# CMU-Perceptual-Computing-Lab/caffe_rtpose

Measured on AMD Instinct MI355X. Metric: frames/sec (whole node) at 656x368 COCO model, higher is better.
Workload: dtype f16; 1 GPU; COCO 656x368, 1 scale(s), synthetic 720p video: pageable host u8 1280x720 frames through rtp_submit_frame: pinned copy + H2D + device warp / INTER_AREA / normalise / pad inside the timed region -> conv stack+ImResize+NMS+connect -> joints on the host; precision mode mixed, 7 frames in flight/GPU in ; precision=mixed, input=host_u8, batch_frames=2, frames_in_flight=7, num_scales=1, exec=graph, hw_queues=4, parallelism=frame-sharded replicas x1

## Files before the change

### caffe_rtpose_amd/csrc/conv_first.hip

```cpp
#include "conv_common.h"

namespace rtp {

namespace {
constexpr int FIRST_ZERO_SLOT = 8;
}

__global__ __launch_bounds__(256) void conv_first_kernel(FirstParams Q) {
  const KStamp kstamp_(Q.stamp);
  extern __shared__ __attribute__((aligned(16))) unsigned char smem_first[];
  _Float16* tile = (_Float16*)smem_first;
  const int W = Q.g.W, H = Q.g.H, TW = W + 2, TW3 = TW * 3;
  const int n = blockIdx.x / H, y = blockIdx.x - n * H;
  const int tid = threadIdx.x, lane = tid & 63, wave = tid >> 6;
  const int lpx = lane & 31, h = lane >> 5;
  const int zero_at = 3 * TW3;

  uint4 wa[2][2];
#pragma unroll
  for (int t = 0; t < 2; ++t)
#pragma unroll
    for (int j = 0; j < 2; ++j) wa[t][j] = Q.wfrag[(t * 2 + j) * 64 + lane];
  floatx16 bz[2];
#pragma unroll
  for (int t = 0; t < 2; ++t)
#pragma unroll
    for (int u = 0; u < 4; ++u) {
      const floatx4 b4 = *(const floatx4*)(Q.bias + t * 32 + (u >> 1) * 16 + h * 8 + (u & 1) * 4);
      bz[t][4 * u] = b4[0]; bz[t][4 * u + 1] = b4[1]; bz[t][4 * u + 2] = b4[2]; bz[t][4 * u + 3] = b4[3];
    }

  const float* img = Q.in + (long)n * 3 * H * W;
  for (int idx = tid; idx < 9 * W; idx += 256) {
    const int rc = idx / W, x = idx - rc * W;
    const int r = rc / 3, c = rc - r * 3;
    const int yy = y + r - 1;
    const float v = (yy >= 0 && yy < H) ? img[((long)c * H + yy) * W + x] : 0.f;
    tile[(r * TW + x + 1) * 3 + c] = (_Float16)v;
  }
  if (tid < 18) {
    const int r = tid / 6, rem = tid - r * 6, side = rem / 3, c = rem - side * 3;
    tile[(r * TW + (side ? W + 1 : 0)) * 3 + c] = (_Float16)0.f;
  }
  if (tid < FIRST_ZERO_SLOT) tile[zero_at + tid] = (_Float16)0.f;
  __syncthreads();

  int off[2][8], mul[2][8];
#pragma unroll
  for (int j = 0; j < 2; ++j)
#pragma unroll
    for (int e2 = 0; e2 < 8; ++e2) {
      const int k = j * 16 + h * 8 + e2;
      const bool real = k < 27;
      off[j][e2] = real ? (k / 9) * TW3 + (k % 9) : zero_at;
      mul[j][e2] = real ? 3 : 0;
    }

  _Float16* orow = Q.out + (((long)n * Q.g.Hp + y + Q.g.halo) * Q.g.Wp + Q.g.halo) * Q.Cp;
  for (int x0 = wave * 32; x0 < W; x0 += 128) {
    const int x = x0 + lpx;
    const int xr = x < W ? x : W - 1;
    half8_t b[2];
#pragma unroll
    for (int j = 0; j < 2; ++j)
#pragma unroll
      for (int e2 = 0; e2 < 8; ++e2) b[j][e2] = tile[xr * mul[j][e2] + off[j][e2]];
    floatx16 acc[2];
#pragma unroll
    for (int t = 0; t < 2; ++t) {
      acc[t] = __builtin_amdgcn_mfma_f32_32x32x16_f16(__builtin_bit_cast(half8_t, wa[t][0]), b[0], bz[t], 0, 0, 0);
      acc[t] = __builtin_amdgcn_mfma_f32_32x32x16_f16(__builtin_bit_cast(half8_t, wa[t][1]), b[1], acc[t], 0, 0, 0);
    }
    if (x < W) {
      _Float16* op = orow + (long)x * Q.Cp;
#pragma unroll
      for (int t = 0; t < 2; ++t)
#pragma unroll
        for (int g = 0; g < 2; ++g) {
          half8_t o;
#pragma unroll
          for (int u = 0; u < 8; ++u) {
            float v = acc[t][g * 8 + u];
            if (Q.relu) v = v > 0.f ? v : 0.f;
            o[u] = (_Float16)v;
          }
          *(half8_t*)(op + t * 32 + g * 16 + h * 8) = o;
        }
    }
  }
}

hipError_t launch_conv_first(const FirstParams& Q, hipStream_t stream) {
  const size_t lds = ((size_t)3 * (Q.g.W + 2) * 3 + FIRST_ZERO_SLOT) * sizeof(_Float16);
  if (lds > 64 * 1024) return hipErrorInvalidValue;
  hipLaunchKernelGGL(conv_first_kernel, dim3(Q.g.N * Q.g.H), dim3(256), lds, stream, Q);
  return hipGetLastError();
}

int conv_first_channel_of_row(int i) {
  const int hh = (i >> 2) & 1, q = (i & 3) + 4 * (i >> 3);
  return (q >> 3) * 16 + hh * 8 + (q & 7);
}

}
```

### caffe_rtpose_amd/csrc/engine.cpp

```cpp
#include <hip/hip_runtime.h>

#include <algorithm>
#include <atomic>
#include <chrono>
#include <cmath>
#include <cstdarg>
#include <cstdio>
#include <cstring>
#include <deque>
#include <fstream>
#include <map>
#include <mutex>
#include <sstream>
#include <string>
#include <thread>
#include <vector>

#include "../../include/rtpose_mi355x.h"
#include "jpeg_plan.h"
#include "kernels.h"
#include "netdef.h"
#include "plan.h"

using namespace rtp;
// ... 260 lines not shown
    for (int n = 0; n < c.cout; ++n) (*out_b)[n] = b[n];
    return;
  }
  if (c.fused) {
    const int rows = c.fused == 1 ? 128 : 64;
    const int parts = c.split_w ? 2 : 1;
    for (int n = 0; n < c.cout; ++n)
      for (int cr = 0; cr < c.cin; ++cr) {
        const int ci = ti.chmap[cr];
        const int chunk = c.fused == 1 ? n / 128 : ci / 128;
        const int row = c.fused == 1 ? n % 128 : n;
        const int k = ci % 128;
        const float wv = w[(size_t)n * c.cin + cr];
        const T hi = (T)wv;
        pw[(((size_t)chunk * parts + 0) * rows + row) * 128 + k] = hi;
        if (c.split_w) pw[(((size_t)chunk * parts + 1) * rows + row) * 128 + k] = (T)(wv - (float)hi);
      }
    out_b->assign(c.CoutP, 0.f);
    for (int n = 0; n < c.cout; ++n) (*out_b)[n] = b[n];
    return;
  }
  if (c.first) {
    for (int n = 0; n < c.cout; ++n)
      for (int r = 0; r < 3; ++r)
        for (int s = 0; s < 3; ++s)
          for (int cc = 0; cc < 3; ++cc) {
            const int j = (r * 3 + s) * 3 + cc;
            const int chunk = j / per_chunk, kk = j % per_chunk;
            const float wv = w[((size_t)(n * 3 + cc) * 3 + r) * 3 + s];
            const T hi = (T)wv;
            pw[((size_t)(0 * c.nchunk + chunk) * c.CoutP + n) * per_chunk + kpos(n, kk)] = hi;
            if (c.split_w) pw[((size_t)(0 * c.nchunk + c.ncp + chunk) * c.CoutP + n) * per_chunk + kpos(n, kk)] = (T)(wv - (float)hi);
          }
  } else {
    for (int n = 0; n < c.cout; ++n)
      for (int cr = 0; cr < c.cin; ++cr) {
        const int ci = ti.chmap[cr];
        const int chunk = ci / per_chunk, kk = ci % per_chunk;
        for (int r = 0; r < c.k; ++r)
          for (int s = 0; s < c.k; ++s) {
            const int tap = r * c.k + s;
            const float wv = w[((size_t)(n * c.cin + cr) * c.k + r) * c.k + s];
            const T hi = (T)wv;
            const T lo = (T)(wv - (float)hi);
            if (c.h8) {
              const size_t tile0 = (size_t)(r * c.nchunk + chunk) * c.k + s;
              pw[(tile0 * c.CoutP + n) * per_chunk + kpos(n, kk)] = hi;
              const size_t tileq = (size_t)(r * c.nchunk + c.ncp + chunk) * c.k + s;
              unsigned char* qrow = out_w->data() + (tileq * c.CoutP + n) * c.rowb;
              const int g = kk / 64, pos = kk % 64;
              auto qpos = [&](int byte) { return ((byte / 16) ^ conv_ring_swz(c.rowb, n)) * 16 + byte % 16; };
              qrow[qpos(g * 128 + pos)] = f32_to_e4m3(std::ldexp((float)hi, c.wq_exp));
              qrow[qpos(g * 128 + 64 + pos)] = f32_to_e4m3(std::ldexp(wv - (float)hi, c.wq_exp + 11));
              continue;
            }
            int vbase = 0;
            for (int pass = 0; pass < 3; ++pass) {
              if ((pass == 1 && !c.split_a) || (pass == 2 && !c.split_w)) continue;
              const int vchunk = vbase + chunk;
              vbase += c.ncp;
              const size_t tile = c.impl == 1 ? ((size_t)(r * c.nchunk + vchunk) * c.k + s) : ((size_t)tap * c.nchunk + vchunk);
              pw[(tile * c.CoutP + n) * per_chunk + kpos(n, kk)] = pass == 2 ? lo : hi;
            }
          }
      }
  }
  out_b->assign(c.CoutP, 0.f);
  for (int n = 0; n < c.cout; ++n) (*out_b)[n] = b[n];
}

void compute_wq_exp(rtp_engine* e) {
  for (auto& s : e->plan.steps) {
    if (s.type != 1 || !e->plan.convs[s.a].h8) continue;
    float mx = 0.f;
    for (int idx : {s.a, s.b}) if (idx >= 0) for (float v : e->w_ref[idx]) mx = std::max(mx, std::fabs(v));
    int ex = mx > 0.f ? (int)std::floor(std::log2(448.0 / mx)) : 0;
    ex = std::max(-20, std::min(ex, 40));
    for (int idx : {s.a, s.b}) if (idx >= 0) e->plan.convs[idx].wq_exp = ex;
  }
}

int upload_conv_weights(rtp_engine* e, int i) {
  const ConvOp& c = e->plan.convs[i];
  std::vector<unsigned char> pw;
  std::vector<float> pb;
  if (e->plan.prec == 0) pack_conv<_Float16>(e->plan, c, e->w_ref[i], e->b_ref[i], &pw, &pb);
  else pack_conv<float>(e->plan, c, e->w_ref[i], e->b_ref[i], &pw, &pb);
  SYNC_GUARD;
  HIPCHK(e, hipMemcpy(e->dweights + c.w_off, pw.data(), pw.size(), hipMemcpyHostToDevice));
  HIPCHK(e, hipMemcpy(e->dweights + c.b_off, pb.data(), pb.size() * sizeof(float), hipMemcpyHostToDevice));
  return RTP_OK;
}

int upload_all_weights(rtp_engine* e) {
  std::vector<unsigned char> image(e->plan.weights_bytes, 0);
  const int n = (int)e->plan.convs.size();
  const int nthr = std::max(1, std::min({(int)std::thread::hardware_concurrency(), 16, n}));
  std::atomic<int> next{0};
  auto work = [&]() {
    std::vector<unsigned char> pw;
    std::vector<float> pb;
    for (int i = next.fetch_add(1); i < n; i = next.fetch_add(1)) {
      const ConvOp& c = e->plan.convs[i];
      if (e->plan.prec == 0) pack_conv<_Float16>(e->plan, c, e->w_ref[i], e->b_ref[i], &pw, &pb);
      else pack_conv<float>(e->plan, c, e->w_ref[i], e->b_ref[i], &pw, &pb);
      memcpy(image.data() + c.w_off, pw.data(), pw.size());
      memcpy(image.data() + c.b_off, pb.data(), pb.size() * sizeof(float));
    }
  };
  std::vector<std::thread> pool;
  for (int t = 1; t < nthr; ++t) pool.emplace_back(work);
  work();
  for (auto& t : pool) t.join();
  SYNC_GUARD;
  HIPCHK(e, hipMemcpy(e->dweights, image.data(), e->plan.weights_bytes, hipMemcpyHostToDevice));
  return RTP_OK;
}

constexpr int STAMP_SLOTS = 256;
unsigned long long* stamp_slot(const rtp_engine* e, const Ctx& cx, int idx) {
  return (e->stamp_probe && cx.stamps && idx >= 0 && idx < STAMP_SLOTS) ? cx.stamps + 2 * (size_t)idx : nullptr;
}
int stamp_harvest(rtp_engine* e, Ctx& cx) {
  if (!cx.stamps || !cx.stamps_dirty) return RTP_OK;
  for (Slot& sl : cx.slot)
    if (sl.export_pending) HIPCHK(e, hipEventSynchronize(sl.ev_export));
  std::vector<unsigned long long> h(2 * STAMP_SLOTS);
  HIPCHK(e, hipMemcpy(h.data(), cx.stamps, h.size() * sizeof(unsigned long long), hipMemcpyDeviceToHost));
  HIPCHK(e, hipMemset(cx.stamps, 0, h.size() * sizeof(unsigned long long)));
  cx.stamps_dirty = false;
  for (int i = 0; i < STAMP_SLOTS; ++i) {
    if (!h[2 * i + 1] || !h[2 * i]) continue;
    const unsigned long long t0 = ~h[2 * i], t1 = h[2 * i + 1];
    if (!e->stamp_base) e->stamp_base = t0;
    if (e->stamp_spans.size() < 3 * (size_t)(1 << 20)) {
      e->stamp_spans.push_back((float)i);
      e->stamp_spans.push_back((float)((double)((long long)(t0 - e->stamp_base)) * 0.01));
      e->stamp_spans.push_back((float)((double)((long long)(t1 - e->stamp_base)) * 0.01));
    }
  }
  return RTP_OK;
}

void fill_problem(const rtp_engine* e, const Ctx& cx, const ConvOp& c, ConvProblem* pr) {
  memset(pr, 0, sizeof(*pr));
  pr->in = cx.arena + e->plan.tensors[c.in_tensor].offset;
  pr->w = e->dweights + c.w_off;
  pr->bias = (const float*)(e->dweights + c.b_off);
  pr->ndst = (int)c.dsts.size();
  for (int d = 0; d < pr->ndst; ++d) {
    const Tensor& t = e->plan.tensors[c.dsts[d].first];
    pr->dst[d].base = cx.arena + t.offset;
    pr->dst[d].cstride = t.stride();
    pr->dst[d].coff = c.dsts[d].second;
    pr->dst[d].lo_off = t.lo_off();
    pr->dst[d].q_off = t.q_off();
  }
  if (c.to_lowres) {
    pr->out_nchw = cx.lowres;
    pr->out_C = e->plan.heat_channels;
    pr->out_coff = c.lowres_coff;
  }
  pr->Cout = c.cout;
}

unsigned long long* g_clkprobe = nullptr;
int launch_conv_step(rtp_engine* e, Ctx& cx, const Step& s, int nimg) {
  const ConvOp& A = e->plan.convs[s.a];
  const Geom& g = e->plan.geom[A.level];
  ConvParams P;
  memset(&P, 0, sizeof P);
  fill_problem(e, cx, A, &P.prob[0]);
  if (s.b >= 0) fill_problem(e, cx, e->plan.convs[s.b], &P.prob[1]);
  P.H = g.H; P.W = g.W; P.Wp = g.Wp; P.halo = g.halo; P.img_pix = g.img_pix;
  P.in_cstride = e->plan.tensors[A.in_tensor].stride();
  P.nchunk = A.nchunk;
  P.wrap_at = A.wrap_at();
  P.last_phys = A.last_phys();
  {
    const Tensor& tin = e->plan.tensors[A.in_tensor];
    const int qb = tin.q_off() * e->plan.elem;
    P.q_from = A.h8 ? A.ncp : 0;
    P.jump_delta = A.h8 ? qb - (A.ncp - 1) * A.rowb : 0;
    P.row_back = A.h8 ? qb + (A.ncp - 1) * A.rowb : A.last_phys() * A.rowb;
    P.wq_exp = A.wq_exp;
  }
  P.CoutP = A.CoutP;
  P.tiles_per_img = (int)conv_tiles_per_img(e->plan, A);
  if (A.pool >= 0) {
    const Geom& go = e->plan.geom[A.level + 1];
    P.pool = 1;
    P.pool_wq = pool_wq(g, A);
    P.pool_Wp = go.Wp; P.pool_halo = go.halo; P.pool_img_pix = go.img_pix;
  }
  P.relu = A.relu ? 1 : 0;
  P.clkprobe = g_clkprobe;
  P.stamp = stamp_slot(e, cx, (int)(&s - e->plan.steps.data()));
  P.nimg = nimg;
  {
    static const char* rot = RTP_EXP_ENV("RTP_CONV_ROTATE");
    P.rotate = (rot && rot[0] == '0') ? 0 : 1;
    static const char* xm = RTP_EXP_ENV("RTP_CONV_XCDMAP");
    P.xcdmap = xm ? atoi(xm) : 1;
    static const char* sb = RTP_EXP_ENV("RTP_RING_SB");
    P.ring_sb = sb ? atoi(sb) : 6;
    static const char* sp = RTP_EXP_ENV("RTP_RING_SPEC");
    P.spec = (sp && sp[0] == '0') ? 0 : 1;
    static const char* rv = RTP_EXP_ENV("RTP_RING_VAR");
    P.variant = rv ? atoi(rv) : 0;
    static const char* ed = RTP_EXP_ENV("RTP_EPI_DIAG");
    P.diag = ed ? atoi(ed) : 0;
    static const char* il = RTP_EXP_ENV("RTP_RING_ILV");
    P.ilv = il ? (il[0] == '1' || (il[0] == 'q' && A.h8) || (il[0] == '7' && A.h8 && A.k_eff == 7)) : (A.h8 ? 1 : 0);
  }
  if (A.impl == 1) HIPCHK(e, launch_conv_ring(e->plan.prec, A.cfg, A.k_eff, A.rowb, P, s.b >= 0 ? 2 : 1, nimg, cx.stream));
  else HIPCHK(e, launch_conv(e->plan.prec, A.cfg, A.k_eff, A.rowb, P, s.b >= 0 ? 2 : 1, nimg, cx.stream));
  return RTP_OK;
}

int launch_pw2_step(rtp_engine* e, Ctx& cx, const Step& s, int nimg) {
  const ConvOp& A = e->plan.convs[s.a];
  const ConvOp& C = e->plan.convs[s.a2];
  const Geom& g = e->plan.geom[C.level];
  Pw2Params Q;
  memset(&Q, 0, sizeof Q);
  ConvParams& P = Q.P2;
  fill_problem(e, cx, C, &P.prob[0]);
  if (s.b2 >= 0) fill_problem(e, cx, e->plan.convs[s.b2], &P.prob[1]);
  P.H = g.H; P.W = g.W; P.Wp = g.Wp; P.halo = g.halo; P.img_pix = g.img_pix;
  P.CoutP = 64;
  P.tiles_per_img = (int)plain_tiles_per_img(g, 64);
  P.relu = C.relu ? 1 : 0;
  P.stamp = stamp_slot(e, cx, (int)(&s - e->plan.steps.data()));
  P.nimg = nimg;
  const int firsts[2] = {s.a, s.b};
  for (int q = 0; q < 2; ++q) {
    if (firsts[q] < 0) continue;
    const ConvOp& F = e->plan.convs[firsts[q]];
    const Tensor& ti = e->plan.tensors[F.in_tensor];
    const Tensor& tm = e->plan.tensors[F.dsts[0].first];
    Q.x_in[q] = cx.arena + ti.offset;
    Q.x_cstride = ti.stride();
    Q.x_lo_off = F.split_a ? ti.lo_off() : 0;
    Q.w1[q] = e->dweights + F.w_off;
    Q.b1[q] = (const float*)(e->dweights + F.b_off);
    Q.mid[q].base = tm.written ? cx.arena + tm.offset : nullptr;
    Q.mid[q].cstride = tm.stride();
    Q.mid[q].coff = 0;
    Q.mid[q].lo_off = tm.lo_off();
  }
  Q.c1_chunks = A.fused_chunks;
  Q.relu1 = A.relu ? 1 : 0;
  Q.split_w1 = A.split_w ? 1 : 0;
  Q.split_w2 = C.split_w ? 1 : 0;
  Q.h_lo = C.split_a ? 1 : 0;
  static const char* probe = RTP_EXP_ENV("RTP_PW2_PROBE");
  static int probed = 0;
  hipStreamCaptureStatus cst = hipStreamCaptureStatusNone;
  if (probe) (void)hipStreamIsCapturing(cx.stream, &cst);
  if (probe && cst == hipStreamCaptureStatusNone && probed < 16) {
    unsigned long long* d = nullptr;
    HIPCHK(e, hipMalloc((void**)&d, 32 * 8));
    HIPCHK(e, hipMemset(d, 0, 32 * 8));
    P.clkprobe = d;
    const auto t0 = std::chrono::steady_clock::now();
    HIPCHK(e, launch_conv_pw2(Q, s.b >= 0 ? 2 : 1, nimg, cx.stream));
    HIPCHK(e, hipStreamSynchronize(cx.stream));
    const double host_us = std::chrono::duration<double, std::micro>(std::chrono::steady_clock::now() - t0).count();
    unsigned long long h[32];
    HIPCHK(e, hipMemcpy(h, d, sizeof h, hipMemcpyDeviceToHost));
    (void)hipFree(d);
    fprintf(stderr, "pw2 probe %s chunks %d splits %d%d%d%d (launch+sync %.1f us): ", A.name.c_str(), Q.c1_chunks, Q.x_lo_off ? 1 : 0, Q.split_w1, Q.h_lo, Q.split_w2, host_us);
    for (unsigned i = 2; i <= h[0] && i < 32; ++i) fprintf(stderr, "%.2f ", (double)(h[i] - h[i - 1]) / 100.0);
    fprintf(stderr, "us; total %.2f us\n", (double)(h[h[0]] - h[1]) / 100.0);
    ++probed;
    return RTP_OK;
  }
  HIPCHK(e, launch_conv_pw2(Q, s.b >= 0 ? 2 : 1, nimg, cx.stream));
  return RTP_OK;
}

}

namespace {
bool is_dominant_class(const rtp_engine* e, const Step& s) {
  if (s.type != 1 || e->plan.dominant_step < 0) return false;
  const ConvOp& a = e->plan.convs[s.a];
  const ConvOp& d = e->plan.convs[e->plan.steps[e->plan.dominant_step].a];
  return a.k == d.k && a.cin == d.cin && a.cout == d.cout && (s.b >= 0) == (e->plan.steps[e->plan.dominant_step].b >= 0);
}

int launch_first_step(rtp_engine* e, Ctx& cx, const Step& s, const float* input_dev, int nimg) {
  const ConvOp& c = e->plan.convs[s.a];
  const Tensor& to = e->plan.tensors[c.dsts[0].first];
  FirstParams Q;
  Q.in = input_dev;
  Q.g = e->plan.geom[0];
  Q.g.N = nimg;
  Q.wfrag = (const uint4*)(e->dweights + c.w_off);
  Q.bias = (const float*)(e->dweights + c.b_off);
  Q.out = (_Float16*)(cx.arena + to.offset);
  Q.Cp = to.stride();
  Q.relu = c.relu ? 1 : 0;
  Q.stamp = stamp_slot(e, cx, (int)(&s - e->plan.steps.data()));
  HIPCHK(e, launch_conv_first(Q, cx.stream));
  return RTP_OK;
}

int run_frame_stack(rtp_engine* e, Ctx& cx, const float* input_dev, int nimg, bool cap = false) {
  const std::vector<PoolOp>& pools = e->plan.pools;
  auto geom_n = [&](int level) { Geom g = e->plan.geom[level]; g.N = nimg; return g; };
  for (size_t si = 0; si < e->plan.steps.size(); ++si) {
    const Step& s = e->plan.steps[si];
    const bool want_timed = e->time_dominant && !cap && nimg == e->plan.NI && (e->time_all || is_dominant_class(e, s));
    const bool timed = want_timed && e->tev_next < (int)e->tev.size() / 2;
    if (want_timed && !timed) e->probe_dropped[0]++;
    if (timed) HIPCHK(e, hipEventRecord(e->tev[2 * (size_t)e->tev_next], cx.stream));
    struct Close {
      rtp_engine* e; Ctx& cx; const Step& s; size_t si; bool timed;
      ~Close() {
        if (!timed) return;
        (void)hipEventRecord(e->tev[2 * (size_t)e->tev_next + 1], cx.stream);
        e->tev_step[e->tev_next] = (short)si;
        e->tev_pass[e->tev_next++] = (unsigned char)(s.type == 1 ? e->plan.convs[s.a].passes() : 1);
      }
    } close_{e, cx, s, si, timed};
    if (s.type == 0) {
      const Tensor& t = e->plan.tensors[0];
      HIPCHK(e, launch_pack_input(e->plan.prec, input_dev, cx.arena + t.offset, geom_n(0), t.stride(), cx.stream));
    } else if (s.type == 1) {
      const int rc = launch_conv_step(e, cx, s, nimg);
      if (rc) return rc;
    } else if (s.type == 3) {
      const int rc = launch_pw2_step(e, cx, s, nimg);
      if (rc) return rc;
    } else if (s.type == 4) {
      const int rc = launch_first_step(e, cx, s, input_dev, nimg);
      if (rc) return rc;
    } else {
      const PoolOp& p = pools[s.a];
      const Tensor& ti = e->plan.tensors[p.in_tensor];
      const Tensor& to = e->plan.tensors[p.out_tensor];
      HIPCHK(e, launch_maxpool(e->plan.prec, cx.arena + ti.offset, geom_n(ti.level), ti.stride(), cx.arena + to.offset, geom_n(to.level), to.stride(),
                               round_up(p.C, 16 / e->plan.elem), ti.lo_off(), to.lo_off(), ti.q_off(), to.q_off(), cx.stream));
    }
  }
  return RTP_OK;
}

ResizeParams resize_params(rtp_engine* e, Ctx& cx, int sj) {
  Slot& sl = cx.slot[sj];
  ResizeParams rp;
  rp.src = cx.lowres + (size_t)sj * e->N * e->plan.heat_channels * e->plan.low_h * e->plan.low_w;
  rp.dst = sl.resized; rp.num = e->N; rp.C = e->plan.heat_channels;
  rp.h = e->plan.low_h; rp.w = e->plan.low_w; rp.tw = e->cfg.net_w; rp.th = e->cfg.net_h;
  rp.start_scale = e->start_scale; rp.scale_gap = e->scale_gap;
  return rp;
}
int run_resize(rtp_engine* e, Ctx& cx, int sj = 0) {
  HIPCHK(e, launch_resize(resize_params(e, cx, sj), cx.slot[sj].stream));
  return RTP_OK;
}
NmsParams nms_params(rtp_engine* e, Ctx& cx, int sj) {
  Slot& sl = cx.slot[sj];
  NmsParams np;
  np.src = sl.resized; np.peaks = sl.peaks; np.strip_count = sl.strip_count; np.strip_list = sl.strip_list;
  np.src_planes = e->plan.heat_channels; np.H = e->cfg.net_h; np.W = e->cfg.net_w; np.num_parts = e->plan.num_parts;
  np.max_peaks = e->plan.max_peaks; np.nstrips = e->plan.nstrips; np.strip_rows = e->plan.strip_rows; np.threshold = e->nms_threshold;
  np.probe = nullptr;
  np.clear_flag = nullptr;
  np.stamp = stamp_slot(e, cx, 64 + 8 * sj);
  return np;
}
int run_nms(rtp_engine* e, Ctx& cx, int sj = 0) {
  HIPCHK(e, launch_nms(nms_params(e, cx, sj), cx.slot[sj].stream));
  return RTP_OK;
}
ConnectParams connect_params(rtp_engine* e, Ctx& cx, int sj) {
  Slot& sl = cx.slot[sj];
  ConnectParams cp;
  memset(&cp, 0, sizeof cp);
  cp.heat = sl.resized; cp.peaks = sl.peaks; cp.joints = sl.joints; cp.num_people = sl.num_people;
  cp.cand_score = sl.cand_score; cp.cand_ij = sl.cand_ij; cp.cand_count = sl.cand_count; cp.cand_blk = sl.cand_blk;
  cp.conn = sl.conn; cp.conn_score = sl.conn_score; cp.conn_count = sl.conn_count;
  cp.max_rows = e->plan.max_rows; cp.model = e->plan.model; cp.num_parts = e->plan.num_parts; cp.num_limbs = e->plan.num_limbs;
  cp.max_peaks = e->plan.max_peaks; cp.net_w = e->cfg.net_w; cp.net_h = e->cfg.net_h; cp.disp_w = e->cfg.disp_w; cp.disp_h = e->cfg.disp_h;
  cp.inter_threshold = e->inter_threshold; cp.inter_min_above = e->inter_min_above; cp.min_subset_cnt = e->min_subset_cnt;
  cp.min_subset_score = e->min_subset_score; cp.max_people = RTP_MAX_PEOPLE;
  cp.stamp = stamp_slot(e, cx, 64 + 8 * sj + 2);
  {
    static const char* pf = RTP_EXP_ENV("RTP_PAIRS_FULL");
    cp.pairs_full = (pf && pf[0] == '1') ? 1 : 0;
  }
  return cp;
}
int run_connect(rtp_engine* e, Ctx& cx, int sj = 0) {
  HIPCHK(e, launch_connect(connect_params(e, cx, sj), cx.slot[sj].stream));
  return RTP_OK;
}
int run_post_fused(rtp_engine* e, Ctx& cx, int sj, hipEvent_t ev_nms) {
  Slot& sl = cx.slot[sj];
  const ResizeParams rp = resize_params(e, cx, sj);
  NmsParams np = nms_params(e, cx, sj);
  np.clear_flag = sl.num_people;
  HIPCHK(e, launch_nms_fused(np, rp, sl.stream));
  HIPCHK(e, hipEventRecord(ev_nms, sl.stream));
  ConnectParams cp = connect_params(e, cx, sj);
  cp.counter_cleared = 1;
  cp.tickets = e->chain_connect ? sl.tickets : nullptr;
  HIPCHK(e, launch_connect_fused(cp, rp, sl.stream));
  return RTP_OK;
}

int jpeg_alloc(rtp_engine* e, int w, int h, JpegBufs* b, unsigned char** host, unsigned char** host_dev, size_t* cap);
void jd_free(JdBufs* b);
int jd_launch(rtp_engine* e, unsigned long long* stamp, const JdJob& job, const FrameView& dst, hipStream_t stream);

int launch_batch_body(rtp_engine* e, Ctx& cx, int nframes, const float* input_dev, bool materialize, bool cap, int part = 3) {
  int rc;
  if (part & 1) {
    HIPCHK(e, hipEventRecord(cx.ev[0], cx.stream));
    if ((rc = run_frame_stack(e, cx, input_dev, nframes * e->N, cap))) return rc;
  }
  if (!(part & 2)) return RTP_OK;
  HIPCHK(e, hipEventRecord(cx.ev[1], cx.stream));
  const size_t jbytes = (size_t)RTP_MAX_PEOPLE * e->plan.num_parts * 3 * sizeof(float);
  for (int j = 0; j < nframes; ++j) {
    Slot& sl = cx.slot[j];
    if (sl.stream != cx.stream) HIPCHK(e, hipStreamWaitEvent(sl.stream, cx.ev[1], 0));
    static const char* diag = RTP_EXP_ENV("RTP_DIAG_SKIP_POST");
    const int skip = diag ? atoi(diag) : 0;
    static const char* unf = RTP_EXP_ENV("RTP_POST_UNFUSED");
    HIPCHK(e, hipEventRecord(sl.ev[0], sl.stream));
    if (skip >= 3) {
      const ResizeParams rp = resize_params(e, cx, j);
      HIPCHK(e, hipEventRecord(sl.ev[1], sl.stream));
      HIPCHK(e, launch_nms_fused(nms_params(e, cx, j), rp, sl.stream));
      HIPCHK(e, hipEventRecord(sl.ev[2], sl.stream));
      if (skip >= 4) {
        ConnectParams cp = connect_params(e, cx, j);
        cp.diag_stages = skip - 3;
        HIPCHK(e, launch_connect_fused(cp, rp, sl.stream));
      }
    } else if (materialize || skip || (unf && unf[0] == '1')) {
      if (skip < 2 && (rc = run_resize(e, cx, j))) return rc;
      HIPCHK(e, hipEventRecord(sl.ev[1], sl.stream));
      if (skip < 2 && (rc = run_nms(e, cx, j))) return rc;
      HIPCHK(e, hipEventRecord(sl.ev[2], sl.stream));
      if (skip < 1 && (rc = run_connect(e, cx, j))) return rc;
    } else {
      HIPCHK(e, hipEventRecord(sl.ev[1], sl.stream));
      if ((rc = run_post_fused(e, cx, j, sl.ev[2]))) return rc;
    }
    HIPCHK(e, hipEventRecord(sl.ev[3], sl.stream));
    if (e->cfg.render && sl.has_disp) {
      const size_t dbytes = (size_t)e->cfg.disp_w * e->cfg.disp_h * 3;
      if (!sl.render_dev) {
        SYNC_GUARD;
        HIPCHK(e, hipMalloc((void**)&sl.render_dev, dbytes));
        HIPCHK(e, hipHostMalloc((void**)&sl.render_host, dbytes, hipHostMallocDefault));
        HIPCHK(e, hipMalloc((void**)&sl.render_tab, render_tab_floats(RTP_MAX_PEOPLE) * sizeof(float)));
      }
      if (e->cfg.render == 1) {
        RenderParams rp;
        rp.src = sl.disp_cur; rp.dst = sl.render_dev; rp.w = e->cfg.disp_w; rp.h = e->cfg.disp_h;
        rp.poses = sl.joints; rp.num_people = sl.num_people; rp.tab = sl.render_tab;
        rp.model = e->plan.model; rp.googly = 0; rp.max_people = RTP_MAX_PEOPLE;
        HIPCHK(e, launch_render(rp, sl.stream));
      } else {
        if (!(materialize || skip || (unf && unf[0] == '1')) && (rc = run_resize(e, cx, j))) return rc;
        RenderViewParams vp;
        vp.src = sl.disp_cur; vp.dst = sl.render_dev; vp.w = e->cfg.disp_w; vp.h = e->cfg.disp_h;
        vp.maps = sl.resized; vp.net_w = e->cfg.net_w; vp.net_h = e->cfg.net_h;
        vp.model = e->plan.model; vp.part_to_show = e->cfg.render - 1;
        HIPCHK(e, launch_render_view(vp, sl.stream));
      }
      if (e->jpeg_quality) {
        if (!sl.jpeg.base) {
          SYNC_GUARD;
          if ((rc = jpeg_alloc(e, e->cfg.disp_w, e->cfg.disp_h, &sl.jpeg, &sl.jpeg_host, &sl.jpeg_host_dev, &sl.jpeg_cap))) return rc;
        }
        const FrameView fv = {sl.render_dev, e->cfg.disp_w, e->cfg.disp_h, 3L * e->cfg.disp_w, 3L, {0L, 1L, 2L}};
        HIPCHK(e, launch_jpeg_encode(stamp_slot(e, cx, 64 + 8 * j + 6), fv, e->jpeg_q, sl.jpeg, sl.jpeg_host_dev,
                                     reinterpret_cast<unsigned*>(sl.jpeg_host_dev + sl.jpeg_cap), sl.stream));
      } else {
        if (!sl.render_host) {
          SYNC_GUARD;
          HIPCHK(e, hipHostMalloc((void**)&sl.render_host, dbytes, hipHostMallocDefault));
        }
        HIPCHK(e, hipMemcpyAsync(sl.render_host, sl.render_dev, dbytes, hipMemcpyDeviceToHost, sl.stream));
      }
    }
    HIPCHK(e, hipMemcpyAsync(sl.host_out + 4, sl.joints, jbytes, hipMemcpyDeviceToHost, sl.stream));
    HIPCHK(e, hipMemcpyAsync(sl.host_out, sl.num_people, sizeof(int), hipMemcpyDeviceToHost, sl.stream));
    HIPCHK(e, hipEventRecord(sl.ev[4], sl.stream));
    if (cap && sl.stream != cx.stream) HIPCHK(e, hipStreamWaitEvent(cx.stream, sl.ev[4], 0));
  }
  return RTP_OK;
}

int capture_batch(rtp_engine* e, Ctx& cx, int nframes, hipGraphExec_t* out) {
  SYNC_GUARD;
  hipGraph_t g = nullptr;
  HIPCHK(e, hipStreamBeginCapture(cx.stream, hipStreamCaptureModeThreadLocal));
  const int rc = launch_batch_body(e, cx, nframes, cx.input, false, true, e->graph_post ? 3 : 1);
  const hipError_t s = hipStreamEndCapture(cx.stream, &g);
  if (rc) { if (g) (void)hipGraphDestroy(g); return rc; }
  if (s != hipSuccess || !g) return fail(e, RTP_EHIP, "hipStreamEndCapture failed: %s", hipGetErrorString(s));
  const hipError_t si = hipGraphInstantiate(out, g, nullptr, nullptr, 0);
  (void)hipGraphDestroy(g);
  if (si != hipSuccess) return fail(e, RTP_EHIP, "hipGraphInstantiate failed: %s", hipGetErrorString(si));
  return RTP_OK;
}

int flush_prep(rtp_engine* e, Ctx& cx, bool force);
int launch_batch(rtp_engine* e, Ctx& cx, int nframes, const float* input_dev, bool materialize = false) {
  int rc;
  cx.last_nframes = nframes;
  cx.last_own_input = input_dev == cx.input;
  cx.last_tags.resize(nframes);
  for (int j = 0; j < nframes; ++j) cx.last_tags[j] = cx.slot[j].tag;
  for (Slot& sl : cx.slot)
    if (sl.export_pending) {
      HIPCHK(e, hipStreamWaitEvent(cx.stream, sl.ev_export, 0));
      sl.export_pending = false;
    }
  if (e->prep_defer && (rc = flush_prep(e, cx, true))) return rc;
  if (cx.in_pending) {
    if (cx.in_stream != cx.stream) {
      HIPCHK(e, hipEventRecord(cx.ev_in, cx.in_stream));
      HIPCHK(e, hipStreamWaitEvent(cx.stream, cx.ev_in, 0));
    }
    cx.in_pending = false;
  }
  static const char* diag = RTP_EXP_ENV("RTP_DIAG_SKIP_POST");
  static const char* unf = RTP_EXP_ENV("RTP_POST_UNFUSED");
  const bool graph = e->use_graph && !e->time_dominant && !materialize && input_dev == cx.input && !e->cfg.render && !diag && !unf && nframes <= 16;
  cx.graph_run = graph;
  cx.graph_conv = false;
  if (!graph) {
    if ((rc = launch_batch_body(e, cx, nframes, input_dev, materialize, false))) return rc;
    cx.launched = true;
    return RTP_OK;
  }
  if (!cx.gexec[nframes] && (rc = capture_batch(e, cx, nframes, &cx.gexec[nframes]))) return rc;
  HIPCHK(e, hipEventRecord(cx.gev[0], cx.stream));
  HIPCHK(e, hipGraphLaunch(cx.gexec[nframes], cx.stream));
  if (!e->graph_post) {
    if ((rc = launch_batch_body(e, cx, nframes, cx.input, false, false, 2))) return rc;
    cx.graph_run = false;
    cx.graph_conv = true;
  }
  HIPCHK(e, hipEventRecord(cx.gev[1], cx.stream));
  cx.launched = true;
  return RTP_OK;
}
int enqueue_frame(rtp_engine* e, Ctx& cx, const float* input_dev, bool materialize = false) { return launch_batch(e, cx, 1, input_dev, materialize); }

int hw_queue_count() {
  const char* v = getenv("GPU_MAX_HW_QUEUES");
  const int q = v ? atoi(v) : 4;
  return q >= 1 && q <= 64 ? q : 4;
}
hipError_t make_stream(hipStream_t* s, bool post) {
#ifdef RTP_EXPERIMENTS
  if (post) {
    const char* c = getenv("RTP_POST_CUS");
    const int n = c ? atoi(c) : 0;
    if (n > 0 && n < 256) {
      uint32_t mask[8] = {0, 0, 0, 0, 0, 0, 0, 0};
      for (int b = 0; b < n; ++b) mask[b >> 5] |= 1u << (b & 31);
      return hipExtStreamCreateWithCUMask(s, 8, mask);
    }
  }
  const char* v = getenv(post ? "RTP_POST_PRIO" : "RTP_CONV_PRIO");
  if (v && v[0]) {
    int least = 0, greatest = 0;
    (void)hipDeviceGetStreamPriorityRange(&least, &greatest);
    int pr = atoi(v);
    pr = std::max(greatest, std::min(least, pr));
    return hipStreamCreateWithPriority(s, hipStreamNonBlocking, pr);
  }
#endif
  (void)post;
  return hipStreamCreateWithFlags(s, hipStreamNonBlocking);
}

size_t staged_yuv_bytes(int w, int h, int sx, int sy, size_t* planes_off) {
  const size_t off = round_up_sz((size_t)w * h * 3, 256);
  if (planes_off) *planes_off = off;
  return off + (size_t)w * h + 2 * (size_t)((w + sx) >> sx) * (size_t)((h + sy) >> sy);
}

int alloc_slot(rtp_engine* e, Ctx& cx, Slot& sl, bool share_stream) {
  if (sl.preset_stream) {}
  else if (share_stream) sl.stream = cx.stream;
  else { HIPCHK(e, make_stream(&sl.stream, true)); sl.own_stream = true; }
  const size_t res_floats = (size_t)e->plan.heat_channels * e->cfg.net_h * e->cfg.net_w;
  HIPCHK(e, hipMalloc((void**)&sl.resized, res_floats * sizeof(float)));
  const size_t peak_floats = (size_t)e->plan.num_parts * (e->plan.max_peaks + 1) * 3;
  HIPCHK(e, hipMalloc((void**)&sl.peaks, peak_floats * sizeof(float)));
  HIPCHK(e, hipMemset(sl.peaks, 0, peak_floats * sizeof(float)));
  HIPCHK(e, hipMalloc((void**)&sl.strip_count, (size_t)e->plan.num_parts * e->plan.nstrips * sizeof(int)));
  HIPCHK(e, hipMalloc((void**)&sl.strip_list, (size_t)e->plan.num_parts * e->plan.nstrips * e->plan.max_peaks * sizeof(int)));
  const size_t pairs = (size_t)e->plan.num_limbs * e->plan.max_peaks * e->plan.max_peaks;
  HIPCHK(e, hipMalloc((void**)&sl.cand_score, pairs * sizeof(float)));
// ... 2573 lines not shown
```

### caffe_rtpose_amd/csrc/kernels.h

```cpp
#pragma once
#include <hip/hip_runtime.h>
#include <stdint.h>
#include <stdlib.h>

#include "jpeg_bound.h"
#include "jpeg_dec.h"

#ifdef RTP_EXPERIMENTS
#define RTP_EXP_ENV(name) getenv(name)
#else
#define RTP_EXP_ENV(name) ((const char*)nullptr)
#endif

namespace rtp {

#if defined(__HIPCC__)
struct KStamp {
  unsigned long long* s;
  __device__ __forceinline__ explicit KStamp(unsigned long long* p) : s(p) {
    if (s && threadIdx.x == 0 && threadIdx.y == 0) atomicMax(s, ~wall_clock64());
  }
  __device__ __forceinline__ ~KStamp() {
    if (s && threadIdx.x == 0 && threadIdx.y == 0) atomicMax(s + 1, wall_clock64());
  }
};
#endif

struct Geom {
  int N, H, W, halo, Hp, Wp;
  long img_pix;
};

#define RTP_MAX_DST 6
struct ConvDst {
  void* base;
  int cstride;
  int coff;
  int lo_off;
  int q_off;
};

struct ConvProblem {
  const void* in;
  const void* w;
  const float* bias;
  ConvDst dst[RTP_MAX_DST];
  int ndst;
  float* out_nchw;
  int out_C, out_coff;
  int Cout;
};

struct ConvParams {
  ConvProblem prob[2];
  int H, W, Wp, halo;
  long img_pix;
  int in_cstride;
  int nchunk;
  int wrap_at;
  int last_phys;
  int q_from;
  int wq_exp;
  int jump_delta;
  int row_back;
  int CoutP;
  int tiles_per_img;
  int nimg;
  int relu;
  int rotate;
  int xcdmap;
  int ring_sb;
  int spec;
  int variant;
  int ilv;
  int pool, pool_wq, pool_Wp, pool_halo;
  long pool_img_pix;
  int diag;
  unsigned long long* stamp;
  unsigned long long* clkprobe;
};

enum ConvCfg { CFG_128x128 = 0, CFG_64x128 = 1, CFG_64x64 = 2, CFG_128x64 = 3, CFG_128x32 = 4, CFG_256x64 = 5, CFG_COUNT = 6 };

struct ConvCfgInfo { int BM, BN; };
inline ConvCfgInfo conv_cfg_info(int cfg) {
  switch (cfg) {
    case CFG_128x128: return {128, 128};
    case CFG_64x128: return {64, 128};
    case CFG_64x64: return {64, 64};
    case CFG_128x32: return {128, 32};
    case CFG_256x64: return {256, 64};
    default: return {128, 64};
  }
}

hipError_t launch_conv(int prec, int cfg, int ks, int rowb, const ConvParams& P, int nprob, int N,
                       hipStream_t stream);

hipError_t launch_conv_ring(int prec, int cfg, int ks, int chb, const ConvParams& P, int nprob, int N,
                            hipStream_t stream);
struct Pw2Params {
  ConvParams P2;
  const void* x_in[2];
  int x_cstride, x_lo_off;
  const void* w1[2];
  const float* b1[2];
  ConvDst mid[2];
  int c1_chunks;
  int relu1;
  int split_w1, split_w2, h_lo;
};
hipError_t launch_conv_pw2(const Pw2Params& Q, int nprob, int nimg, hipStream_t stream);

inline int conv_ring_swz(int chb, int row) { return chb == 256 ? (row & 15) : ((row >> 1) & 7); }

hipError_t launch_pack_input(int prec, const float* in_nchw, void* out, Geom g, int Cp, hipStream_t stream);
struct FirstParams {
  const float* in;
  Geom g;
  const uint4* wfrag;
  const float* bias;
  _Float16* out;
  int Cp;
  int relu;
  unsigned long long* stamp;
};
hipError_t launch_conv_first(const FirstParams& Q, hipStream_t stream);
int conv_first_channel_of_row(int i);
hipError_t launch_maxpool(int prec, const void* in, Geom gi, int Cpi, void* out, Geom go, int Cpo, int C, int lo_i, int lo_o, int q_i, int q_o,
                          hipStream_t stream);
hipError_t launch_export(int prec, const void* in, Geom g, int Cp, const int* chmap_dev, int C, int lo_off, int q_off, float* out,
                         hipStream_t stream);

struct AreaScale {
  int tw, th, identity;
  int fast_x, fast_y;
  const int* xstart; const int* xsi; const float* xalpha;
  const int* ystart; const int* ysi; const float* yalpha;
  int linear;
  const int* lx; const int* ly;
};
hipError_t launch_warp(unsigned long long* stamp, const unsigned char* src, int sw, int sh, double inv, const short* tab2d, unsigned char* dst, int dw, int dh,
                       hipStream_t stream);
hipError_t launch_area_pad(unsigned long long* stamp, const unsigned char* disp, int dw, int dh, const AreaScale* scales, int nscales, float* out, int net_w, int net_h,
                           hipStream_t stream);

struct FrameView {
  unsigned char* data;
  int w, h;
  long row, pix;
  long off[3];
};
enum FrameLayout { LAYOUT_GENERIC = 0, LAYOUT_HWC3_BGR, LAYOUT_HWC3_RGB, LAYOUT_HWC4_BGR, LAYOUT_HWC4_RGB, LAYOUT_PLANAR };
int frame_layout(const FrameView& v, size_t avail);
hipError_t launch_frame_import(unsigned long long* stamp, const FrameView& v, int layout, unsigned char* dst, hipStream_t stream);
hipError_t launch_frame_export(unsigned long long* stamp, const unsigned char* src, const FrameView& v, int layout, hipStream_t stream);
hipError_t launch_warp_view(unsigned long long* stamp, const FrameView& v, double inv, const short* tab2d, unsigned char* dst, int dw, int dh,
                            hipStream_t stream);

struct YuvView {
  const unsigned char* y;
  const unsigned char* u;
  const unsigned char* v;
  int w, h, sx, sy;
  long ys, uvs, uvp;
};
enum YuvLayout { YUV_GENERIC = 0, YUV_420_PLANAR, YUV_420_NV12, YUV_420_NV21 };
int yuv_layout(const YuvView& s, const FrameView& d);
inline FrameView packed_bgr_view(unsigned char* p, int w, int h) { return FrameView{p, w, h, 3L * w, 3, {0, 1, 2}}; }
hipError_t launch_yuv_import(unsigned long long* stamp, const YuvView& s, const FrameView& d, int layout, hipStream_t stream);

struct JpegHuffTab { unsigned short code[256]; unsigned char size[256]; };
struct JpegQuant { unsigned recip[2][64]; unsigned short half[2][64]; };
struct JpegBufs {
  void* base = nullptr;
  int w = 0, h = 0;
  JpegHuffTab* huff = nullptr;
  short* coef = nullptr;
  unsigned* bits = nullptr;
  unsigned* mcubits = nullptr;
  unsigned* off = nullptr;
  int* dcdiff = nullptr;
  unsigned* words = nullptr;
  unsigned* counts = nullptr;
  unsigned* meta = nullptr;
  unsigned char* data = nullptr;
};
size_t jpeg_bufs_bytes(int w, int h, JpegBufs* layout);
hipError_t launch_jpeg_encode(unsigned long long* stamp, const FrameView& v, const JpegQuant& q, const JpegBufs& jb, unsigned char* dst,
                              unsigned* dst_len, hipStream_t stream);

struct JdTables { JdScan scan; JdHuff dc[3], ac[3]; };
struct JdLayout {
  size_t words = 0, tab = 0, segs = 0, subs = 0, staged = 0;
  size_t entry = 0, exit_ = 0, count = 0, excl = 0, gexit = 0, flags = 0, status = 0, coef = 0, dcsum = 0, planes = 0, total = 0;
  int ngroups = 0;
};
JdLayout jd_layout(long blocks, long plane_bytes, size_t nwords, size_t nsegs, size_t nsubs, int group);
struct JdDev {
  const JdTables* tab;
  const JdSeg* segs;
  const JdSub* subs;
  const uint32_t* words;
  int nsub, nwords, ngroups;
  JdState* entry;
  JdState* exit_;
  int* count;
  int* excl;
  JdState* gexit;
  int* flags;
  unsigned* status;
  unsigned* status_out;
  short* coef;
  int* dcsum;
};
struct JdRecon {
  int W, H, ncomp, rgb, hmax, vmax, blocks;
  int h[3], v[3], bw[3], bh[3], dw[3], dh[3], coef_off[3];
  long plane_off[3];
  unsigned short qn[3][64];
};
hipError_t launch_jpeg_entropy(unsigned long long* stamp, const JdDev& d, int group, int mcus, int ncomp, long blocks, hipStream_t stream);
hipError_t launch_jpeg_reconstruct(unsigned long long* stamp, const JdRecon& g, const short* coef, unsigned char* planes, const FrameView& dv, hipStream_t stream);

struct RenderParams {
  const unsigned char* src;
  unsigned char* dst;
  int w, h;
  const float* poses;
  const int* num_people;
  float* tab;
  int model, googly, max_people;
};
hipError_t launch_render(const RenderParams& p, hipStream_t stream);
size_t render_tab_floats(int max_people);
struct RenderViewParams {
  const unsigned char* src;
  unsigned char* dst;
  int w, h;
  const float* maps;
  int net_w, net_h;
  int model, part_to_show;
};
hipError_t launch_render_view(const RenderViewParams& p, hipStream_t stream);

struct ResizeParams {
  const float* src;
  float* dst;
  int num, C, h, w, tw, th;
  float start_scale, scale_gap;
};
hipError_t launch_resize(const ResizeParams& p, hipStream_t stream);

struct NmsParams {
  const float* src;
  float* peaks;
  int* strip_count;
  int* strip_list;
  int src_planes, H, W, num_parts, max_peaks, nstrips, strip_rows;
  float threshold;
  unsigned long long* probe;
  unsigned long long* stamp;
  int* clear_flag;
};
hipError_t launch_nms(const NmsParams& p, hipStream_t stream);
hipError_t launch_nms_fused(const NmsParams& p, const ResizeParams& r, hipStream_t stream);

struct ConnectParams {
  unsigned long long* stamp;
  int counter_cleared;
  int* tickets;
  const float* heat;
  const float* peaks;
  float* joints;
  int* num_people;
  float* cand_score;
  int* cand_ij;
  int* cand_count;
  int* cand_blk;
  int* conn;
  float* conn_score;
  int* conn_count;
  int* subset_idx;
  double* subset_score;
  int* subset_cnt;
  int max_rows;
  int assemble_preload;
  int pairs_full;
  int diag_stages;
  int model;
  int num_parts, num_limbs, max_peaks;
  int net_w, net_h, disp_w, disp_h;
  float inter_threshold;
  int inter_min_above;
  int min_subset_cnt;
  float min_subset_score;
  int max_people;
};
hipError_t launch_connect(const ConnectParams& p, hipStream_t stream);
hipError_t launch_connect_fused(const ConnectParams& p, const ResizeParams& r, hipStream_t stream);

}
```

Measured before the change: 1071 frames/s.

## Rework first conv: vectorized tile load, packed im2col, LDS-transposed coalesced stores

Rewrites the first 3x3 conv kernel. The input tile is now loaded with float4 reads of all three channels and stored as packed 4-half pixels. The B fragments are built from 9 uint2 LDS reads with bit shuffles instead of 16 scalar gathered loads. Output goes through a per-wave swizzled LDS transpose so each global store writes a full 128-byte pixel row contiguously, and ReLU is templated and done on packed halves. Adds experiment-only variants behind an env var, which needs more LDS and the W%4==0 restriction.

Result: no change. 1084 frames/s, median of 6 (+1.2%).

```diff
diff --git a/caffe_rtpose_amd/csrc/conv_first.hip b/caffe_rtpose_amd/csrc/conv_first.hip
--- a/caffe_rtpose_amd/csrc/conv_first.hip
+++ b/caffe_rtpose_amd/csrc/conv_first.hip
@@ -1,12 +1,155 @@
+#include <atomic>
+
 #include "conv_common.h"
 
 namespace rtp {
 
 namespace {
+constexpr int FIRST_TR_BYTES = 4 * 32 * 128;
+constexpr int FIRST_LDS_MAX = 160 * 1024;
+
+typedef _Float16 first_h2 __attribute__((ext_vector_type(2)));
+__device__ __forceinline__ unsigned first_pack2(float a, float b) {
+  first_h2 v;
+  v[0] = (_Float16)a; v[1] = (_Float16)b;
+  return __builtin_bit_cast(unsigned, v);
+}
+template <bool RELU> __device__ __forceinline__ unsigned first_out2(float a, float b) {
+  first_h2 v;
+  v[0] = (_Float16)a; v[1] = (_Float16)b;
+  if constexpr (RELU) v = __builtin_elementwise_max(v, (first_h2){(_Float16)0.f, (_Float16)0.f});
+  return __builtin_bit_cast(unsigned, v);
+}
+}
+
+template <int VAR, bool RELU>
+__global__ __launch_bounds__(256) void conv_first_kernel(FirstParams Q) {
+  const KStamp kstamp_(Q.stamp);
+  extern __shared__ __attribute__((aligned(16))) unsigned char smem_first[];
+  const int W = Q.g.W, H = Q.g.H, TW = W + 2;
+  const int n = blockIdx.x / H, y = blockIdx.x - n * H;
+  const int tid = threadIdx.x, lane = tid & 63, wave = tid >> 6;
+  const int lpx = lane & 31, h = lane >> 5;
+  unsigned char* trbuf = smem_first + wave * (32 * 128);
+  uint2* tile = (uint2*)(smem_first + FIRST_TR_BYTES);
+  _Float16* orow = Q.out + (((long)n * Q.g.Hp + y + Q.g.halo) * Q.g.Wp + Q.g.halo) * Q.Cp;
+  const int spx = lane >> 3, spiece = lane & 7;
+  const unsigned char* tr_rd = trbuf + spx * 128 + ((spiece ^ spx) << 4);
+
+  if constexpr (VAR == 2) {
+    for (int x0 = wave * 32; x0 < W; x0 += 128)
+#pragma unroll
+      for (int k = 0; k < 4; ++k) {
+        const int x = x0 + 8 * k + spx;
+        if (x < W) *(uint4*)(orow + (long)x * Q.Cp + spiece * 8) = make_uint4(0, 0, 0, 0);
+      }
+    return;
+  }
+
+  uint4 wa[2][2];
+#pragma unroll
+  for (int t = 0; t < 2; ++t)
+#pragma unroll
+    for (int j = 0; j < 2; ++j) wa[t][j] = Q.wfrag[(t * 2 + j) * 64 + lane];
+  floatx16 bz[2];
+#pragma unroll
+  for (int t = 0; t < 2; ++t)
+#pragma unroll
+    for (int u = 0; u < 4; ++u) {
+      const floatx4 b4 = *(const floatx4*)(Q.bias + t * 32 + (u >> 1) * 16 + h * 8 + (u & 1) * 4);
+      bz[t][4 * u] = b4[0]; bz[t][4 * u + 1] = b4[1]; bz[t][4 * u + 2] = b4[2]; bz[t][4 * u + 3] = b4[3];
+    }
+
+  if constexpr (VAR != 4) {
+    const float* img = Q.in + (long)n * 3 * H * W;
+    const long plane = (long)H * W;
+#pragma unroll
+    for (int r = 0; r < 3; ++r) {
+      const int yy = y + r - 1;
+      const bool in = yy >= 0 && yy < H;
+      const float* src = img + (long)(in ? yy : 0) * W;
+      uint2* trow = tile + r * TW + 1;
+      for (int q = tid; q < (W >> 2); q += 256) {
+        floatx4 c0 = {0.f, 0.f, 0.f, 0.f}, c1 = c0, c2 = c0;
+        if (in) {
+          c0 = *(const floatx4*)(src + 4 * q);
+          c1 = *(const floatx4*)(src + plane + 4 * q);
+          c2 = *(const floatx4*)(src + 2 * plane + 4 * q);
+        }
+#pragma unroll
+        for (int i = 0; i < 4; ++i) trow[4 * q + i] = make_uint2(first_pack2(c0[i], c1[i]), first_pack2(c2[i], 0.f));
+      }
+    }
+    if (tid < 6) tile[(tid >> 1) * TW + ((tid & 1) ? W + 1 : 0)] = make_uint2(0, 0);
+  }
+  __syncthreads();
+
+  for (int x0 = wave * 32; x0 < W; x0 += 128) {
+    const int x = x0 + lpx;
+    const int xr = x < W ? x : W - 1;
+    uint4 b[2];
+    if constexpr (VAR == 3) {
+      b[0] = make_uint4(0x3c003c00u, 0x3c003c00u, 0x3c003c00u, 0x3c003c00u);
+      b[1] = b[0];
+    } else {
+      const uint2* px = tile + xr;
+      uint2 P[3][3];
+#pragma unroll
+      for (int r = 0; r < 3; ++r)
+#pragma unroll
+        for (int s = 0; s < 3; ++s) P[r][s] = px[r * TW + s];
+      const unsigned d0 = P[0][0].x;
+      const unsigned d1 = P[0][0].y | (P[0][1].x << 16);
+      const unsigned d2 = __builtin_amdgcn_alignbit(P[0][1].y, P[0][1].x, 16);
+      const unsigned d3 = P[0][2].x;
+      const unsigned d4 = P[0][2].y | (P[1][0].x << 16);
+      const unsigned d5 = __builtin_amdgcn_alignbit(P[1][0].y, P[1][0].x, 16);
+      const unsigned d6 = P[1][1].x;
+      const unsigned d7 = P[1][1].y | (P[1][2].x << 16);
+      const unsigned d8 = __builtin_amdgcn_alignbit(P[1][2].y, P[1][2].x, 16);
+      const unsigned d9 = P[2][0].x;
+      const unsigned d10 = P[2][0].y | (P[2][1].x << 16);
+      const unsigned d11 = __builtin_amdgcn_alignbit(P[2][1].y, P[2][1].x, 16);
+      const unsigned d12 = P[2][2].x;
+      const unsigned d13 = P[2][2].y;
+      b[0] = h ? make_uint4(d4, d5, d6, d7) : make_uint4(d0, d1, d2, d3);
+      b[1] = h ? make_uint4(d12, d13, 0u, 0u) : make_uint4(d8, d9, d10, d11);
+    }
+    floatx16 acc[2];
+#pragma unroll
+    for (int t = 0; t < 2; ++t) {
+      acc[t] = __builtin_amdgcn_mfma_f32_32x32x16_f16(__builtin_bit_cast(half8_t, wa[t][0]), __builtin_bit_cast(half8_t, b[0]), bz[t], 0, 0, 0);
+      acc[t] = __builtin_amdgcn_mfma_f32_32x32x16_f16(__builtin_bit_cast(half8_t, wa[t][1]), __builtin_bit_cast(half8_t, b[1]), acc[t], 0, 0, 0);
+    }
+#pragma unroll
+    for (int t = 0; t < 2; ++t)
+#pragma unroll
+      for (int g = 0; g < 2; ++g) {
+        uint4 o;
+        const float* v = (const float*)&acc[t] + g * 8;
+        o.x = first_out2<RELU>(v[0], v[1]); o.y = first_out2<RELU>(v[2], v[3]); o.z = first_out2<RELU>(v[4], v[5]); o.w = first_out2<RELU>(v[6], v[7]);
+        const int piece = t * 4 + g * 2 + h;
+        *(uint4*)(trbuf + lpx * 128 + ((piece ^ (lpx & 7)) << 4)) = o;
+      }
+    asm volatile("" ::: "memory");
+    __builtin_amdgcn_wave_barrier();
+    asm volatile("" ::: "memory");
+#pragma unroll
+    for (int k = 0; k < 4; ++k) {
+      const uint4 v = *(const uint4*)(tr_rd + k * 1024);
+      const int xs = x0 + 8 * k + spx;
+      if (VAR != 1 && xs < W) *(uint4*)(orow + (long)xs * Q.Cp + spiece * 8) = v;
+      if constexpr (VAR == 1) asm volatile("" :: "v"(v.x), "v"(v.y), "v"(v.z), "v"(v.w));
+    }
+    asm volatile("" ::: "memory");
+    __builtin_amdgcn_wave_barrier();
+    asm volatile("" ::: "memory");
+  }
+}
+
+#ifdef RTP_EXPERIMENTS
 constexpr int FIRST_ZERO_SLOT = 8;
-}
-
-__global__ __launch_bounds__(256) void conv_first_kernel(FirstParams Q) {
+__global__ __launch_bounds__(256) void conv_first_kernel_r06(FirstParams Q) {
   const KStamp kstamp_(Q.stamp);
   extern __shared__ __attribute__((aligned(16))) unsigned char smem_first[];
   _Float16* tile = (_Float16*)smem_first;
@@ -90,11 +233,47 @@
   }
 }
 
-hipError_t launch_conv_first(const FirstParams& Q, hipStream_t stream) {
+static hipError_t first_launch_r06(const FirstParams& Q, hipStream_t stream) {
   const size_t lds = ((size_t)3 * (Q.g.W + 2) * 3 + FIRST_ZERO_SLOT) * sizeof(_Float16);
   if (lds > 64 * 1024) return hipErrorInvalidValue;
-  hipLaunchKernelGGL(conv_first_kernel, dim3(Q.g.N * Q.g.H), dim3(256), lds, stream, Q);
+  hipLaunchKernelGGL(conv_first_kernel_r06, dim3(Q.g.N * Q.g.H), dim3(256), lds, stream, Q);
   return hipGetLastError();
+}
+#endif
+
+static size_t conv_first_lds_bytes(int W) { return FIRST_TR_BYTES + (size_t)3 * (W + 2) * 4 * sizeof(_Float16); }
+
+template <int VAR, bool RELU>
+static hipError_t first_launch(const FirstParams& Q, hipStream_t stream) {
+  auto kern = conv_first_kernel<VAR, RELU>;
+  const size_t lds = conv_first_lds_bytes(Q.g.W);
+  if (lds > FIRST_LDS_MAX || (Q.g.W & 3)) return hipErrorInvalidValue;
+  if (lds > 64 * 1024) {
+    static std::atomic<unsigned> attr_mask{0};
+    int dev = 0;
+    (void)hipGetDevice(&dev);
+    if (!(attr_mask.load(std::memory_order_relaxed) & (1u << (dev & 31)))) {
+      hipError_t e = hipFuncSetAttribute((const void*)kern, hipFuncAttributeMaxDynamicSharedMemorySize, FIRST_LDS_MAX);
+      if (e != hipSuccess) return e;
+      attr_mask.fetch_or(1u << (dev & 31), std::memory_order_relaxed);
+    }
+  }
+  hipLaunchKernelGGL(kern, dim3(Q.g.N * Q.g.H), dim3(256), lds, stream, Q);
+  return hipGetLastError();
+}
+
+hipError_t launch_conv_first(const FirstParams& Q, hipStream_t stream) {
+#ifdef RTP_EXPERIMENTS
+  switch (Q.variant) {
+    case 1: return first_launch<1, true>(Q, stream);
+    case 2: return first_launch<2, true>(Q, stream);
+    case 3: return first_launch<3, true>(Q, stream);
+    case 4: return first_launch<4, true>(Q, stream);
+    case 9: return first_launch_r06(Q, stream);
+    default: break;
+  }
+#endif
+  return Q.relu ? first_launch<0, true>(Q, stream) : first_launch<0, false>(Q, stream);
 }
 
 int conv_first_channel_of_row(int i) {
diff --git a/caffe_rtpose_amd/csrc/engine.cpp b/caffe_rtpose_amd/csrc/engine.cpp
--- a/caffe_rtpose_amd/csrc/engine.cpp
+++ b/caffe_rtpose_amd/csrc/engine.cpp
@@ -586,6 +586,8 @@
   Q.out = (_Float16*)(cx.arena + to.offset);
   Q.Cp = to.stride();
   Q.relu = c.relu ? 1 : 0;
+  static const char* fv = RTP_EXP_ENV("RTP_FIRST_VAR");
+  Q.variant = fv ? atoi(fv) : 0;
   Q.stamp = stamp_slot(e, cx, (int)(&s - e->plan.steps.data()));
   HIPCHK(e, launch_conv_first(Q, cx.stream));
   return RTP_OK;
diff --git a/caffe_rtpose_amd/csrc/kernels.h b/caffe_rtpose_amd/csrc/kernels.h
--- a/caffe_rtpose_amd/csrc/kernels.h
+++ b/caffe_rtpose_amd/csrc/kernels.h
@@ -123,6 +123,7 @@
   _Float16* out;
   int Cp;
   int relu;
+  int variant;
   unsigned long long* stamp;
 };
 hipError_t launch_conv_first(const FirstParams& Q, hipStream_t stream);
```
